# excamera/alfalfa

Hardware: AMD Instinct MI355X
Metric: 1080p macroblocks/s decode (bit-exact vs reference) (higher is better)
Workload: dtype u8

## Files before the change

__graft_entry__.py:

```python
import os
import subprocess
import sys

ROOT = os.path.dirname(os.path.abspath(__file__))
for p in (ROOT, os.path.join(ROOT, "oracle")):
    if p not in sys.path:
        sys.path.insert(0, p)


def build():
    from alfalfa_amd import build as b
    b.build(force=True, verbose=True)
    subprocess.run(["make", "-C", os.path.join(ROOT, "oracle"), "liboracle.so"], check=True)
    if os.path.isdir("/root/reference/src/decoder"):
        subprocess.run(["make", "-j8", "-C", os.path.join(ROOT, "oracle"), "ref"], check=True)
    import alfalfa_amd
    from alfalfa_amd import capi
    capi.lib()
    dont_write = sys.dont_write_bytecode
    sys.dont_write_bytecode = True
    try:
        sys.path.insert(0, os.path.join(ROOT, "tests"))
        import test_gpu_stages
        test_gpu_stages.build_stage_lib()
        if os.path.isdir("/root/reference/src/frontend"):
            import test_reference_callers as rc
            rc.build_callers(); rc.build_state_check(); rc.build_two_step()
    finally:
        sys.dont_write_bytecode = dont_write


def smoke():
    import alfalfa_amd as aa
    import vp8_oracle as vo
    path = os.path.join(ROOT, "tests", "golden", "qcif_q30_lf24.ivf")
    w, h, frames = aa.read_ivf(path)
    ctx = aa.Context(0)
    dec = aa.Decoder(ctx, w, h)
    ora = vo.OracleDecoder(w, h)
    for i, fr in enumerate(frames[:3]):
        shown, fi = dec.get_frame_output(fr)
        ora.decode(fr)
        assert dec.raster_bytes(fi) == ora.raster_bytes(), "HIP path differs from the oracle at frame %d" % i
    print("smoke ok: %d frames, %dx%d, bit-exact vs oracle" % (3, w, h))


if __name__ == "__main__":
    build()
    if "--smoke" in sys.argv:
        smoke()
```

alfalfa_amd/csrc/coeff_pack.hh:

```
#pragma once
#include "tok_fsm.hh"

namespace aa {
namespace pack {

constexpr uint64_t kInvZigzagNib = tok::nib( { 0, 1, 5, 6, 2, 4, 7, 12, 3, 8, 11, 13, 9, 10, 14, 15 } );
constexpr bool inverse_ok()
{
  for ( unsigned k = 0; k < 16; k++ )
    if ( ( ( kInvZigzagNib >> ( 4 * ( ( tok::kZigzagNib >> ( 4 * k ) ) & 15u ) ) ) & 15u ) != k ) return false;
  return true;
}
static_assert( inverse_ok(), "kInvZigzagNib is not the inverse of the zigzag scan" );

AA_HD inline uint32_t popc( uint32_t v )
{
#if defined( __HIP_DEVICE_COMPILE__ )
  return static_cast<uint32_t>( __popc( v ) );
#else
  return static_cast<uint32_t>( __builtin_popcount( v ) );
#endif
}

AA_HD inline uint32_t blocks_of( uint32_t nz_mask ) { return popc( nz_mask & 0x01FFFFFFu ); }

constexpr uint32_t kMaskSlots = 25;
AA_HD inline uint32_t zigzag_of( uint32_t j ) { return static_cast<uint32_t>( kInvZigzagNib >> ( 4 * j ) ) & 15u; }
template <class P> AA_HD inline int16_t value_at( uint32_t mask, P v, uint32_t j )
{
  const uint32_t k = zigzag_of( j );
  if ( !( ( mask >> k ) & 1u ) ) return 0;
  return static_cast<int16_t>( v[popc( mask & ( ( 1u << k ) - 1u ) )] );
}
AA_HD inline uint32_t parse_order_block( uint32_t p ) { return p == 0 ? 24u : p - 1u; }

template <class L> AA_HD inline size_t word_offset( uint32_t pos, L list )
{
  return static_cast<size_t>( list[1u + ( pos >> 15 )] ) * kChunkWords + ( pos & ( kChunkWords - 1u ) );
}

inline uint32_t expand_macroblock( const int16_t * words, uint32_t nz_mask, int16_t * dense )
{
  if ( !( nz_mask & 0x01FFFFFFu ) ) return 0;
  const int16_t * v = words + kMaskSlots;
  uint32_t n = 0;
  for ( uint32_t p = 0; p < 25; p++ ) {
    const uint32_t b = parse_order_block( p );
    if ( !( ( nz_mask >> b ) & 1u ) ) continue;
    const uint32_t mask = static_cast<uint16_t>( words[b] );
    for ( uint32_t j = 0; j < 16; j++ ) dense[16 * n + j] = value_at( mask, v, j );
    v += popc( mask );
    n++;
  }
  return static_cast<uint32_t>( v - words );
}

}
}
```

alfalfa_amd/csrc/kernels.hip:

```cpp
#include <hip/hip_runtime.h>
#include <algorithm>
#include <cstddef>

#include <cstdlib>

#include "device_types.h"
#include "vp8_math.hh"
#include "coeff_pack.hh"
#include "recon_inl.hh"

namespace aa {
namespace {
using namespace recon;

constexpr int kLanes = 64;

enum : int { DC_PRED, V_PRED, H_PRED, TM_PRED, B_PRED, NEARESTMV, NEARMV, ZEROMV, NEWMV, SPLITMV };

struct alignas( 16 ) ResidualLds {
  union {
    int16_t cf[25][16];
    int16_t res[24][16];
  };
  int16_t im[24][16];
// ... 579 lines not shown
    const int gy = cy0 - 4 + r, gx = cx0 - 4 + d * 4;
    uint32_t v = 0;
    if ( gy >= 0 && gx >= 0 ) v = *reinterpret_cast<const uint32_t *>( f.cur[1 + pl] + static_cast<size_t>( gy ) * cw + gx );
    *reinterpret_cast<uint32_t *>( &L.c[pl][r][d * 4] ) = v;
  }
  __syncthreads();

  lf_passes( L, col > 0, row > 0, !( mb.flags & AA_MB_LF_SKIP_INNER ), P, lane );

  for ( int i = lane; i < 100; i += kLanes ) {
    const int r = i / 5, d = i % 5;
    const int gy = y0 - 4 + r, gx = x0 - 4 + d * 4;
    if ( r == 0 || gy < 0 || gx < 0 ) continue;
    if ( r < 4 && d == 0 ) continue;
    *reinterpret_cast<uint32_t *>( Y + static_cast<size_t>( gy ) * pw + gx ) = *reinterpret_cast<const uint32_t *>( &L.y[r][d * 4] );
  }
  for ( int i = lane; i < 72; i += kLanes ) {
    const int pl = i / 36, e = i % 36, r = e / 3, d = e % 3;
    const int gy = cy0 - 4 + r, gx = cx0 - 4 + d * 4;
    if ( r == 0 || gy < 0 || gx < 0 ) continue;
    if ( r < 4 && d == 0 ) continue;
    *reinterpret_cast<uint32_t *>( f.cur[1 + pl] + static_cast<size_t>( gy ) * cw + gx ) = *reinterpret_cast<const uint32_t *>( &L.c[pl][r][d * 4] );
  }
}

struct alignas( 16 ) Intra4Slot {
  alignas( 16 ) int16_t res[24][16];
  alignas( 16 ) uint8_t y[17][48];
  alignas( 16 ) uint8_t c[2][9][32];
  alignas( 16 ) int16_t y2[32];
};
struct alignas( 16 ) Intra4Lds { Intra4Slot slot[4]; uint32_t tab[160]; };

template <class Slot>
__device__ __forceinline__ void residual_x4( Slot & S, const aa_dev_frame & f, const bool has_res, const bool has_y2, const uint32_t nz_mask,
                                             const uint32_t coeff_index, const uint32_t off_hi, const int segment, const int l )
{
  if ( __any( has_res ) ) {
    const bool pk = f.packed != 0;
    const int16_t * const src = pk ? f.coeffs + ( static_cast<size_t>( off_hi ) << 32 | coeff_index ) : f.coeffs + static_cast<size_t>( coeff_index ) * 16;
    const uint16_t * const q = f.quant[segment];
    const bool y2_stored = has_y2 && ( ( nz_mask >> 24 ) & 1u );
    uint32_t vbase = pack::kMaskSlots;
    if ( __any( y2_stored ) ) {
      if ( y2_stored ) {
        if ( pk ) {
          const uint32_t m24 = static_cast<uint16_t>( src[24] );
          const uint32_t zz = pack::zigzag_of( static_cast<uint32_t>( l ) );
          const int c = ( ( m24 >> zz ) & 1u ) ? src[pack::kMaskSlots + __popc( m24 & ( ( 1u << zz ) - 1u ) )] : 0;
          S.y2[l] = static_cast<int16_t>( dequant( c, q[l ? 3 : 2] ) );
          vbase += __popc( m24 );
        } else S.y2[l] = static_cast<int16_t>( dequant( src[l], q[l ? 3 : 2] ) );
      }
      __syncthreads();
      if ( y2_stored && l < 4 ) {
        const Quad v = iwht_pass1( S.y2[l], S.y2[l + 4], S.y2[l + 8], S.y2[l + 12] );
        S.y2[16 + l] = static_cast<int16_t>( v.v0 ); S.y2[16 + l + 4] = static_cast<int16_t>( v.v1 );
        S.y2[16 + l + 8] = static_cast<int16_t>( v.v2 ); S.y2[16 + l + 12] = static_cast<int16_t>( v.v3 );
      }
      __syncthreads();
      if ( y2_stored && l < 4 ) {
        const int o = l * 4;
        const Quad v = iwht_pass2( S.y2[16 + o], S.y2[16 + o + 1], S.y2[16 + o + 2], S.y2[16 + o + 3] );
        S.y2[o] = static_cast<int16_t>( v.v0 ); S.y2[o + 1] = static_cast<int16_t>( v.v1 );
        S.y2[o + 2] = static_cast<int16_t>( v.v2 ); S.y2[o + 3] = static_cast<int16_t>( v.v3 );
      }
      __syncthreads();
    }
#pragma unroll
    for ( int round = 0; round < 2; round++ ) {
      const int blk = round == 0 ? l : 16 + ( l & 7 );
      const bool mine = has_res && ( round == 0 || l < 8 );
      const bool stored = mine && ( ( nz_mask >> blk ) & 1u );
      const bool wht_dc = round == 0 && has_y2;
      const int dc = ( wht_dc && y2_stored ) ? S.y2[blk] : 0;
      if ( !__any( mine ) ) continue;
      if ( __any( stored ) ) {
        uint32_t d[8] = { 0, 0, 0, 0, 0, 0, 0, 0 };
        const uint32_t pmask = ( stored && pk ) ? static_cast<uint16_t>( src[blk] ) : 0u;
        const int pcount = __popc( pmask ), pincl = slot_scan16( pcount );
        if ( __any( stored && pk ) ) load_packed_block( pmask, src + vbase + ( pincl - pcount ), d );
        vbase += static_cast<uint32_t>( __shfl( pincl, 15, 16 ) );
        if ( stored && !pk ) {
          const uint4 * p = reinterpret_cast<const uint4 *>( src + ( __popc( nz_mask & ( ( 1u << blk ) - 1u ) ) + static_cast<int>( nz_mask >> 24 ) ) * 16 );
          const uint4 a = p[0], b = p[1];
          d[0] = a.x; d[1] = a.y; d[2] = a.z; d[3] = a.w; d[4] = b.x; d[5] = b.y; d[6] = b.z; d[7] = b.w;
        }
        const int base = round == 0 ? 0 : 4;
        int r[16];
        idct_block_regs( d, q[base], q[base + 1], wht_dc, dc, r );
        if ( mine ) {
          uint32_t o[8];
#pragma unroll
          for ( int i = 0; i < 8; i++ ) o[i] = ( static_cast<uint32_t>( r[2 * i] ) & 0xFFFFu ) | ( static_cast<uint32_t>( r[2 * i + 1] ) << 16 );
          uint4 * dst = reinterpret_cast<uint4 *>( &S.res[blk][0] );
          dst[0] = make_uint4( o[0], o[1], o[2], o[3] ); dst[1] = make_uint4( o[4], o[5], o[6], o[7] );
        }
      } else if ( mine ) {
        const pk2 v = pk_splat( ( static_cast<int16_t>( dc ) + 4 ) >> 3 );
        uint4 * dst = reinterpret_cast<uint4 *>( &S.res[blk][0] );
        dst[0] = make_uint4( v, v, v, v ); dst[1] = make_uint4( v, v, v, v );
      }
    }
  }
}

__device__ __forceinline__ uint32_t bigpred_x4( const int mode, const uint32_t above, const int left, const int corner, const int dc, const bool has_res, const int16_t * res )
{
  uint32_t out = 0;
#pragma unroll
  for ( int j = 0; j < 4; j++ ) {
    int v = bigpred_pixel( mode, ( above >> ( 8 * j ) ) & 0xFF, left, corner, dc );
    if ( has_res ) v = clamp255( v + res[j] );
    out |= static_cast<uint32_t>( v ) << ( 8 * j );
  }
  return out;
}

__device__ __forceinline__ void recon_intra4_row( const aa_frame_list & list, const int group, const int row, const int mbh_max, aa_sync_ws * ws, Intra4Lds & L,
                                                  const int home_xcc )
{
  const int lane = threadIdx.x, slot = lane >> 4, l = lane & 15;
  Intra4Slot & S = L.slot[slot];
  const aa_dev_frame * const fp = list.f[group * 4 + slot];
  const aa_dev_frame & f = fp ? *fp : *list.f[group * 4];
  const bool frame_on = fp != nullptr && row < fp->mbh;
  const int mbw = f.mbw, pw = mbw * 16, cw = pw >> 1;
  const int y0 = row * 16, cy0 = row * 8;
  int * const progress = ws->progress + ( group * 4 + slot ) * mbh_max;
  uint8_t * const Y = f.cur[0];
  uint8_t * const Cl = f.cur[1 + ( l >> 3 )];
  const int words = ( frame_on && f.has_intra ) ? ( mbw + 63 ) >> 6 : 0;
  const unsigned long long * const mask = f.intra_rows + static_cast<size_t>( row ) * ( ( mbw + 63 ) >> 6 );
  int w = 0;
  unsigned long long m = words ? mask[0] : 0ull;
  bool row_done = false;
  int seen = row > 0 ? 0 : 0x7FFFFFFF;

  for ( ;; ) {
    while ( m == 0 && w + 1 < words ) { ++w; m = mask[w]; }
    const bool on = m != 0;
    if ( !__any( on ) ) break;
    const int col = on ? w * 64 + __ffsll( static_cast<long long>( m ) ) - 1 : 0;
    m &= m - 1;
    publish_progress( frame_on && l == 0 && ( on || !row_done ), &progress[row], on ? col : mbw );
    row_done = row_done || !on;

    const aa_mb_info * const mb = f.mbs + static_cast<size_t>( row ) * mbw + col;
    uint4 hd = make_uint4( 0, 0, 0, 0 ), bm = make_uint4( 0, 0, 0, 0 );
    if ( on ) { hd = *reinterpret_cast<const uint4 *>( mb ); bm = *reinterpret_cast<const uint4 *>( mb->u.b_mode ); }
    const int y_mode = hd.x & 0xFF, uv_mode = ( hd.x >> 8 ) & 0xFF, segment = ( hd.x >> 24 ) & 3, flags = hd.y & 0xFF;
    const uint32_t nz_mask = hd.z, coeff_index = hd.w;
    const bool has_res = on && ( flags & AA_MB_HAS_NONZERO );
    const bool has_y2 = has_res && ( flags & AA_MB_HAS_Y2 );
    const int need = min( col + 2, mbw );
    if ( on && row > 0 && seen < need ) seen = poll_progress( &progress[row - 1] );

    residual_x4( S, f, has_res, has_y2, nz_mask, coeff_index, hd.y >> 24, segment, l );

    if ( row > 0 ) wait_for_row_above( on, need, seen, 1, ws, progress, group, row, mbh_max, home_xcc, kMinPolls, kMaxWaitTicks );
    const int x0 = col * 16, cx0 = col * 8;
    if ( on ) {
      if ( l < 6 ) {
        uint32_t v;
        const uint8_t * a = Y + static_cast<size_t>( y0 - 1 ) * pw;
        if ( y0 == 0 ) v = 0x7F7F7F7Fu;
        else if ( l == 0 ) v = x0 > 0 ? load_u32<true>( a + x0 - 4 ) : 0x81818181u;
        else if ( l <= 4 ) v = load_u32<true>( a + x0 + ( l - 1 ) * 4 );
        else if ( x0 + 16 >= pw ) v = 0x01010101u * ( load_u32<true>( a + pw - 4 ) >> 24 );
        else v = load_u32<true>( a + x0 + 16 );
        *reinterpret_cast<uint32_t *>( &S.y[0][12 + l * 4] ) = v;
      } else if ( l < 12 ) {
        const int pl = ( l - 6 ) / 3, i = ( l - 6 ) % 3;
        const uint8_t * a = f.cur[1 + pl] + static_cast<size_t>( cy0 - 1 ) * cw;
        uint32_t v;
        if ( cy0 == 0 ) v = 0x7F7F7F7Fu;
        else if ( i == 0 ) v = cx0 > 0 ? load_u32<true>( a + cx0 - 4 ) : 0x81818181u;
        else v = load_u32<true>( a + cx0 + ( i - 1 ) * 4 );
        *reinterpret_cast<uint32_t *>( &S.c[pl][0][12 + i * 4] ) = v;
      }
      S.y[l + 1][15] = x0 > 0 ? static_cast<uint8_t>( load_u32<true>( Y + static_cast<size_t>( y0 + l ) * pw + x0 - 4 ) >> 24 ) : 129;
      S.c[l >> 3][( l & 7 ) + 1][15] = cx0 > 0 ? static_cast<uint8_t>( load_u32<true>( Cl + static_cast<size_t>( cy0 + ( l & 7 ) ) * cw + cx0 - 4 ) >> 24 ) : 129;
    }
    __syncthreads();

    if ( on ) {
      const int pl = l >> 3, r = l & 7;
      const uint32_t a0 = *reinterpret_cast<const uint32_t *>( &S.c[pl][0][16] ), a1 = *reinterpret_cast<const uint32_t *>( &S.c[pl][0][20] );
      const int sa = absdiff_sum4( a0 ) + absdiff_sum4( a1 );
      int sl = 0;
#pragma unroll
// ... 64 lines not shown
      packed |= ( idx < 4 ? ( 4 - idx ) * 48 : idx - 4 ) << ( 8 * k );
      packed |= ( idx >= 9 ? 1u : 0u ) << ( 24 + k );
    }
    L.tab[i] = packed;
  }
  const int xcc = xcc_id();
  if ( xcc >= n_xcd ) { if ( threadIdx.x == 0 ) atomicExch( &ws->error, 3 ); return; }
  for ( ;; ) {
    const int t = take_ticket( ws, xcc, &s_ticket, threadIdx.x );
    const int mine = xcc < n_groups ? ( n_groups - xcc + n_xcd - 1 ) / n_xcd : 0;
    if ( t >= mine * mbh_max ) return;
    recon_intra4_row( list, ( t % mine ) * n_xcd + xcc, t / mine, mbh_max, ws, L, xcc );
  }
}

struct alignas( 16 ) Inter4Slot {
  alignas( 16 ) int16_t res[24][16];
  union {
    struct {
      alignas( 16 ) uint8_t wy[21][24];
      uint8_t wc[2][13][16];
    };
    alignas( 16 ) uint8_t pred[384];
  };
  union {
    alignas( 16 ) uint8_t ty[16][24];
    alignas( 16 ) int16_t y2[32];
  };
  alignas( 16 ) uint8_t tc[2][8][16];
};
struct alignas( 16 ) Inter4Lds { Inter4Slot slot[4]; uint32_t taps[16]; };
static_assert( offsetof( Inter4Slot, wc ) == offsetof( Inter4Slot, wy ) + 21 * 24, "wy and wc must be contiguous" );

__device__ __forceinline__ void recon_inter4_body( const aa_dev_frame & f, const unsigned bq, const unsigned max_quads, Inter4Lds & L )
{
  const int lane = threadIdx.x, slot = lane >> 4, l = lane & 15;
  Inter4Slot & S = L.slot[slot];
  if ( lane < 16 ) {
    uint32_t a, b; pack_taps( lane >> 1, a, b ); L.taps[lane] = ( lane & 1 ) ? b : a;
  }
  const unsigned total = static_cast<unsigned>( f.mbw ) * f.mbh;
  const unsigned chunk = ( max_quads + 7u ) >> 3;
  const unsigned qi = ( bq & 7u ) * chunk + ( bq >> 3 );
  const unsigned mi = qi * 4u + slot;
  const int mbw = f.mbw, pw = mbw * 16, ph = f.mbh * 16, cw = pw >> 1, ch = ph >> 1;
  bool on = qi < max_quads && mi < total;
  const aa_mb_info * const mb = f.mbs + ( on ? mi : 0u );
  uint4 hd = make_uint4( 0, 0, 0, 0 ); uint32_t mvw = 0;
  if ( on ) { hd = *reinterpret_cast<const uint4 *>( mb ); mvw = *reinterpret_cast<const uint32_t *>( &mb->u.mv[0][0] ); }
  const int y_mode = hd.x & 0xFF, ref_frame = ( hd.x >> 16 ) & 3, segment = ( hd.x >> 24 ) & 3, flags = hd.y & 0xFF;
  const uint32_t nz_mask = hd.z, coeff_index = hd.w;
  on = on && ( flags & AA_MB_INTER ) && y_mode != SPLITMV;
  if ( !__any( on ) ) return;
  const int col = on ? static_cast<int>( mi % static_cast<unsigned>( mbw ) ) : 0, row = on ? static_cast<int>( mi / static_cast<unsigned>( mbw ) ) : 0;
  const bool has_res = on && ( flags & AA_MB_HAS_NONZERO );
  const bool has_y2 = has_res && ( flags & AA_MB_HAS_Y2 );
  const uint8_t * const * ref = f.ref[on ? ref_frame : 1];
  const uint8_t * const ref_y = ref[0], * const ref_u = ref[1], * const ref_v = ref[2];
  const int mvx = static_cast<int16_t>( mvw & 0xFFFFu ), mvy = static_cast<int>( mvw ) >> 16;
  const int cmx = chroma_mv( 4 * mvx ), cmy = chroma_mv( 4 * mvy );
  const int sxy = col * 16 + ( mvx >> 3 ) - 2, syy = row * 16 + ( mvy >> 3 ) - 2;
  const int sxc = col * 8 + ( cmx >> 3 ) - 2, syc = row * 8 + ( cmy >> 3 ) - 2;
  const int axy = sxy & ~3, axc = sxc & ~3;
  const bool inside = sxy >= 0 && syy >= 0 && axy + 24 <= pw && syy + 21 <= ph && sxc >= 0 && syc >= 0 && axc + 16 <= cw && syc + 13 <= ch;
  const bool fast = on && inside;
  uint32_t wreg[15];
  const int l6 = l / 6, lm = l - 6 * l6;
  const uint8_t * const wy0 = ref_y + static_cast<ptrdiff_t>( syy ) * pw + axy;
  const uint8_t * const wu0 = ref_u + static_cast<ptrdiff_t>( syc ) * cw + axc;
  const uint8_t * const wv0 = ref_v + static_cast<ptrdiff_t>( syc ) * cw + axc;
#pragma unroll
  for ( int k = 0; k < 15; k++ ) {
    const int i = l + 16 * k;
    wreg[k] = 0;
    if ( fast ) {
      if ( k < 7 || ( k == 7 && i < 126 ) ) {
        const int carry = lm + ( 4 * k ) % 6 >= 6 ? 1 : 0;
        const int r = l6 + 2 * k + ( 4 * k ) / 6 + carry, d = lm + ( 4 * k ) % 6 - 6 * carry;
        wreg[k] = *reinterpret_cast<const uint32_t *>( wy0 + static_cast<ptrdiff_t>( r ) * pw + d * 4 );
      } else if ( i < 230 ) {
        const int j = i - 126, pl = j >= 52 ? 1 : 0, e = j - 52 * pl;
        wreg[k] = *reinterpret_cast<const uint32_t *>( ( pl ? wv0 : wu0 ) + static_cast<ptrdiff_t>( e >> 2 ) * cw + ( e & 3 ) * 4 );
      }
    }
  }

  residual_x4( S, f, has_res, has_y2, nz_mask, coeff_index, hd.y >> 24, segment, l );

  {
    uint32_t * flat = reinterpret_cast<uint32_t *>( &S.wy[0][0] );
    if ( fast ) {
#pragma unroll
      for ( int k = 0; k < 15; k++ ) { const int i = l + 16 * k; if ( i < 230 ) flat[i] = wreg[k]; }
    }
    if ( __any( on && !inside ) ) {
      if ( on && !inside ) {
        uint8_t * by = &S.wy[0][0];
        for ( int i = l; i < 21 * 24; i += 16 ) {
          const int r = i / 24, c = i % 24;
          by[i] = ref_y[static_cast<size_t>( clampi( syy + r, 0, ph - 1 ) ) * pw + clampi( sxy + c, 0, pw - 1 )];
        }
        uint8_t * bc = &S.wc[0][0][0];
        for ( int i = l; i < 2 * 13 * 16; i += 16 ) {
          const int pl = i / 208, e = i % 208, r = e >> 4, c = e & 15;
          bc[i] = ( pl ? ref_v : ref_u )[static_cast<size_t>( clampi( syc + r, 0, ch - 1 ) ) * cw + clampi( sxc + c, 0, cw - 1 )];
        }
      }
    }
  }
  const int oy = inside ? ( sxy & 3 ) : 0, oc = inside ? ( sxc & 3 ) : 0;
  __syncthreads();

  const bool luma_general = __any( on && ( ( mvx | mvy ) & 7 ) != 0 ), chroma_general = __any( on && ( ( cmx | cmy ) & 7 ) != 0 );
  const uint8_t * const wyb = &S.wy[0][0]; const uint8_t * const wcb = &S.wc[0][0][0];
  uint8_t * const tyb = &S.ty[0][0]; uint8_t * const tcb = &S.tc[0][0][0];
  if ( on && luma_general ) {
    const int frac = mvx & 7;
    const uint32_t t0 = L.taps[2 * frac], t1 = L.taps[2 * frac + 1];
#pragma unroll
    for ( int k = 0; k < 6; k++ ) {
// ... 44 lines not shown
    const int frac = mvy & 7;
    const uint32_t t0 = L.taps[2 * frac], t1 = L.taps[2 * frac + 1];
#pragma unroll
    for ( int k = 0; k < 4; k++ ) {
      const int t = l + 16 * k, c = t >> 2, i = t & 3;
      const uint8_t * sp = tyb + c * 24 + i * 4;
      const uint32_t o4 = sixtap_x4_lane( *reinterpret_cast<const uint32_t *>( sp ), *reinterpret_cast<const uint32_t *>( sp + 4 ), *reinterpret_cast<const uint32_t *>( sp + 8 ), 0, frac, t0, t1 );
      uint8_t * pb = S.pred + ( i * 4 ) * 16 + c;
      pb[0] = static_cast<uint8_t>( o4 ); pb[16] = static_cast<uint8_t>( o4 >> 8 ); pb[32] = static_cast<uint8_t>( o4 >> 16 ); pb[48] = static_cast<uint8_t>( o4 >> 24 );
    }
  }
  if ( on && chroma_general ) {
    const int frac = cmy & 7;
    const uint32_t t0 = L.taps[2 * frac], t1 = L.taps[2 * frac + 1];
#pragma unroll
    for ( int k = 0; k < 2; k++ ) {
      const int j = l + 16 * k, pl = j >> 4, c = ( j >> 1 ) & 7, i = j & 1;
      const uint8_t * sp = tcb + pl * 128 + c * 16 + i * 4;
      const uint32_t o4 = sixtap_x4_lane( *reinterpret_cast<const uint32_t *>( sp ), *reinterpret_cast<const uint32_t *>( sp + 4 ), *reinterpret_cast<const uint32_t *>( sp + 8 ), 0, frac, t0, t1 );
      uint8_t * pb = S.pred + 256 + pl * 64 + ( i * 4 ) * 8 + c;
      pb[0] = static_cast<uint8_t>( o4 ); pb[8] = static_cast<uint8_t>( o4 >> 8 ); pb[16] = static_cast<uint8_t>( o4 >> 16 ); pb[24] = static_cast<uint8_t>( o4 >> 24 );
    }
  }
  __syncthreads();

  if ( on ) {
    uint32_t o[4];
#pragma unroll
    for ( int k = 0; k < 4; k++ ) {
      const uint32_t p4 = *reinterpret_cast<const uint32_t *>( S.pred + l * 16 + 4 * k );
      const uint32_t out = has_res ? add_residual_x4( p4, &S.res[( l >> 2 ) * 4 + k][( l & 3 ) * 4] ) : p4;
      o[k] = out;
    }
    *reinterpret_cast<uint4 *>( f.cur[0] + static_cast<size_t>( row * 16 + l ) * pw + col * 16 ) = make_uint4( o[0], o[1], o[2], o[3] );
    const int pl = l >> 3, r = l & 7;
    uint32_t oc2[2];
#pragma unroll
    for ( int k = 0; k < 2; k++ ) {
      const uint32_t p4 = *reinterpret_cast<const uint32_t *>( S.pred + 256 + pl * 64 + r * 8 + 4 * k );
      const uint32_t out = has_res ? add_residual_x4( p4, &S.res[16 + pl * 4 + ( r >> 2 ) * 2 + k][( r & 3 ) * 4] ) : p4;
      oc2[k] = out;
    }
    *reinterpret_cast<uint2 *>( f.cur[1 + pl] + static_cast<size_t>( row * 8 + r ) * cw + col * 8 ) = make_uint2( oc2[0], oc2[1] );
  }
}

__global__ __launch_bounds__( kLanes ) void k_recon_inter4( const aa_frame_list list, const unsigned max_quads )
{
  __builtin_amdgcn_s_setprio( 3 );

  __shared__ Inter4Lds L;
  recon_inter4_body( *list.f[blockIdx.y], blockIdx.x, max_quads, L );
}

constexpr int kStripMbs = 8;
constexpr int kStripRow = 16 + 16 * kStripMbs;
constexpr int kStripRpi = 16 / kStripMbs;
static_assert( ( kStripRow / 16 ) % 2 == 1, "odd multiple of 16: consecutive rows start on different banks" );
struct alignas( 16 ) LfStrip {
  uint8_t c[12][kStripRow];
  uint8_t y[20][kStripRow];
  uint8_t halo_y[16][4];
  uint8_t halo_c[2][8][4];
  uint8_t pad[32];
};
struct alignas( 16 ) LfStripLds { LfStrip slot[4]; };

__device__ __forceinline__ uint64_t load_u64_shared( const uint8_t * p )
{
  return __hip_atomic_load( reinterpret_cast<const uint64_t *>( p ), __ATOMIC_RELAXED, __HIP_MEMORY_SCOPE_AGENT );
}

__device__ __forceinline__ void lf_edges_pk( pk2 ( &v )[20], const LfParamsPk & P, const pk2 g0, const pk2 g1, const pk2 g23 )
{
  if ( __any( g0 != 0u ) ) lf_edge_pk( P, true, g0, v[0], v[1], v[2], v[3], v[4], v[5], v[6], v[7] );
  if ( __any( g1 != 0u ) ) {
    lf_edge_pk( P, false, g1, v[4], v[5], v[6], v[7], v[8], v[9], v[10], v[11] );
    if ( __any( g23 != 0u ) ) {
      lf_edge_pk( P, false, g23, v[8], v[9], v[10], v[11], v[12], v[13], v[14], v[15] );
      lf_edge_pk( P, false, g23, v[12], v[13], v[14], v[15], v[16], v[17], v[18], v[19] );
    }
  }
}

__device__ __forceinline__ void loopfilter_strip_row( const aa_frame_list & list, const int group, const int row, const int mbh_max, const int mbw_max,
// ... 479 lines not shown
```

alfalfa_amd/csrc/recon_inl.hh:

```
#pragma once
#include <hip/hip_runtime.h>

#include "vp8_math.hh"
#include "coeff_pack.hh"

namespace aa {
namespace recon {

__device__ __forceinline__ void pack_taps( const int frac, uint32_t & t0123, uint32_t & t45 )
{
  t0123 = ( sixtap_coeff( frac, 0 ) & 0xFF ) | ( ( sixtap_coeff( frac, 1 ) & 0xFF ) << 8 ) | ( ( sixtap_coeff( frac, 2 ) & 0xFF ) << 16 )
          | ( static_cast<uint32_t>( sixtap_coeff( frac, 3 ) & 0xFF ) << 24 );
  t45 = ( sixtap_coeff( frac, 4 ) & 0xFF ) | ( ( sixtap_coeff( frac, 5 ) & 0xFF ) << 8 );
}

__device__ __forceinline__ void idct_block_regs( const uint32_t ( &d )[8], const int fdc, const int fac, const bool replace_dc, const int dc, int ( &r )[16] )
{
  const pk2 fpair = pk_splat( fac ), f0 = ( static_cast<uint32_t>( fdc ) & 0xFFFFu ) | ( static_cast<uint32_t>( fac ) << 16 );
  int c[16];
#pragma unroll
  for ( int i = 0; i < 8; i++ ) {
    const pk2 m = pk_mul( d[i], i == 0 ? f0 : fpair );
    c[2 * i] = static_cast<int16_t>( m & 0xFFFFu ); c[2 * i + 1] = static_cast<int>( m ) >> 16;
  }
  if ( replace_dc ) c[0] = dc;
  int im[16];
#pragma unroll
  for ( int i = 0; i < 4; i++ ) { const Quad v = idct_pass1( c[i], c[i + 4], c[i + 8], c[i + 12] ); im[i * 4] = v.v0; im[i * 4 + 1] = v.v1; im[i * 4 + 2] = v.v2; im[i * 4 + 3] = v.v3; }
#pragma unroll
  for ( int i = 0; i < 4; i++ ) { const Quad v = idct_pass2( im[i], im[i + 4], im[i + 8], im[i + 12] ); r[i * 4] = v.v0; r[i * 4 + 1] = v.v1; r[i * 4 + 2] = v.v2; r[i * 4 + 3] = v.v3; }
}


__device__ __forceinline__ int slot_scan16( int v )
{
  v += __builtin_amdgcn_update_dpp( 0, v, 0x111, 0xF, 0xF, true );
  v += __builtin_amdgcn_update_dpp( 0, v, 0x112, 0xF, 0xF, true );
  v += __builtin_amdgcn_update_dpp( 0, v, 0x114, 0xF, 0xF, true );
  v += __builtin_amdgcn_update_dpp( 0, v, 0x118, 0xF, 0xF, true );
  return v;
}
__device__ __forceinline__ void load_packed_block( const uint32_t mask, const int16_t * const v, uint32_t ( &d )[8] )
{
#pragma unroll
  for ( int j = 0; j < 16; j++ ) {
    const uint32_t zz = static_cast<uint32_t>( pack::kInvZigzagNib >> ( 4 * j ) ) & 15u;
    const bool there = ( mask >> zz ) & 1u;
    if ( !__any( there ) ) continue;
    uint32_t c = 0;
    if ( there ) c = static_cast<uint16_t>( v[__popc( mask & ( ( 1u << zz ) - 1u ) )] );
    d[j >> 1] |= c << ( 16 * ( j & 1 ) );
  }
}


__device__ __forceinline__ uint32_t sixtap_x4_lane( const uint32_t d0, const uint32_t d1, const uint32_t d2, const int o, const int frac, const uint32_t t0123, const uint32_t t45 )
{
  const uint32_t w0 = __builtin_amdgcn_alignbyte( d1, d0, o ), w1 = __builtin_amdgcn_alignbyte( d2, d1, o ), w2 = __builtin_amdgcn_alignbyte( 0u, d2, o );
  const uint32_t ident = __builtin_amdgcn_alignbyte( w1, w0, 2 );
  const uint32_t b0 = w0 ^ 0x80808080u, b1 = w1 ^ 0x80808080u, b2 = w2 ^ 0x80808080u;
  int v[4];
#pragma unroll
  for ( int k = 0; k < 4; k++ ) {
    const int a = static_cast<int>( __builtin_amdgcn_alignbyte( b1, b0, k ) ), b = static_cast<int>( __builtin_amdgcn_alignbyte( b2, b1, k ) );
    v[k] = __builtin_amdgcn_sdot4( a, static_cast<int>( t0123 ), __builtin_amdgcn_sdot4( b, static_cast<int>( t45 ), 16384 + 64, false ), false );
  }
  const uint32_t lo = __builtin_amdgcn_ashr_pk_u8_i32( v[0], v[1], 7 ), hi = __builtin_amdgcn_ashr_pk_u8_i32( v[2], v[3], 7 );
  const uint32_t out = __builtin_amdgcn_perm( hi, lo, 0x05040100u );
  return frac == 0 ? ident : out;
}

__device__ __forceinline__ uint32_t add_residual_x4( const uint32_t p4, const int16_t * res )
{
  const uint2 r = *reinterpret_cast<const uint2 *>( res );
  const pk2 s0 = pk_add( __builtin_amdgcn_perm( 0u, p4, 0x0c010c00u ), r.x ), s1 = pk_add( __builtin_amdgcn_perm( 0u, p4, 0x0c030c02u ), r.y );
  uint32_t b0, b1;
  asm( "v_sat_pk_u8_i16 %0, %1" : "=v"( b0 ) : "v"( s0 ) );
  asm( "v_sat_pk_u8_i16 %0, %1" : "=v"( b1 ) : "v"( s1 ) );
  return b0 | ( b1 << 16 );
}


}
}
// ... 1 lines not shown
```

Measured before the change: 124.9 million.

## Batch residual coefficient loads ahead of Y2 WHT and use wave-held frame descriptor

Restructures residual_x4 so that the luma, chroma and Y2 coefficient masks are fetched early and all coefficient loads for both rounds are issued together before the WHT barriers. This lets global-load latency overlap instead of serialising per round. The inter kernel now loads the frame descriptor with one dword per lane and extracts fields with readlane, and accesses use explicit global address-space pointers. This raises register pressure (two 16-entry coefficient arrays held live) and adds a new test build step.

```diff
diff --git a/__graft_entry__.py b/__graft_entry__.py
--- a/__graft_entry__.py
+++ b/__graft_entry__.py
@@ -23,6 +23,8 @@
         sys.path.insert(0, os.path.join(ROOT, "tests"))
         import test_gpu_stages
         test_gpu_stages.build_stage_lib()
+        import test_gpu_residual_loads
+        test_gpu_residual_loads.build_residual_stage_lib()
         if os.path.isdir("/root/reference/src/frontend"):
             import test_reference_callers as rc
             rc.build_callers(); rc.build_state_check(); rc.build_two_step()
diff --git a/alfalfa_amd/csrc/coeff_pack.hh b/alfalfa_amd/csrc/coeff_pack.hh
--- a/alfalfa_amd/csrc/coeff_pack.hh
+++ b/alfalfa_amd/csrc/coeff_pack.hh
@@ -32,6 +32,12 @@
   if ( !( ( mask >> k ) & 1u ) ) return 0;
   return static_cast<int16_t>( v[popc( mask & ( ( 1u << k ) - 1u ) )] );
 }
+constexpr uint32_t kNoValue = 0xFFFFFFFFu;
+AA_HD inline uint32_t value_index( uint32_t mask, uint32_t j )
+{
+  const uint32_t k = zigzag_of( j );
+  return ( ( mask >> k ) & 1u ) ? popc( mask & ( ( 1u << k ) - 1u ) ) : kNoValue;
+}
 AA_HD inline uint32_t parse_order_block( uint32_t p ) { return p == 0 ? 24u : p - 1u; }
 
 template <class L> AA_HD inline size_t word_offset( uint32_t pos, L list )
diff --git a/alfalfa_amd/csrc/kernels.hip b/alfalfa_amd/csrc/kernels.hip
--- a/alfalfa_amd/csrc/kernels.hip
+++ b/alfalfa_amd/csrc/kernels.hip
@@ -635,79 +635,6 @@
 };
 struct alignas( 16 ) Intra4Lds { Intra4Slot slot[4]; uint32_t tab[160]; };
 
-template <class Slot>
-__device__ __forceinline__ void residual_x4( Slot & S, const aa_dev_frame & f, const bool has_res, const bool has_y2, const uint32_t nz_mask,
-                                             const uint32_t coeff_index, const uint32_t off_hi, const int segment, const int l )
-{
-  if ( __any( has_res ) ) {
-    const bool pk = f.packed != 0;
-    const int16_t * const src = pk ? f.coeffs + ( static_cast<size_t>( off_hi ) << 32 | coeff_index ) : f.coeffs + static_cast<size_t>( coeff_index ) * 16;
-    const uint16_t * const q = f.quant[segment];
-    const bool y2_stored = has_y2 && ( ( nz_mask >> 24 ) & 1u );
-    uint32_t vbase = pack::kMaskSlots;
-    if ( __any( y2_stored ) ) {
-      if ( y2_stored ) {
-        if ( pk ) {
-          const uint32_t m24 = static_cast<uint16_t>( src[24] );
-          const uint32_t zz = pack::zigzag_of( static_cast<uint32_t>( l ) );
-          const int c = ( ( m24 >> zz ) & 1u ) ? src[pack::kMaskSlots + __popc( m24 & ( ( 1u << zz ) - 1u ) )] : 0;
-          S.y2[l] = static_cast<int16_t>( dequant( c, q[l ? 3 : 2] ) );
-          vbase += __popc( m24 );
-        } else S.y2[l] = static_cast<int16_t>( dequant( src[l], q[l ? 3 : 2] ) );
-      }
-      __syncthreads();
-      if ( y2_stored && l < 4 ) {
-        const Quad v = iwht_pass1( S.y2[l], S.y2[l + 4], S.y2[l + 8], S.y2[l + 12] );
-        S.y2[16 + l] = static_cast<int16_t>( v.v0 ); S.y2[16 + l + 4] = static_cast<int16_t>( v.v1 );
-        S.y2[16 + l + 8] = static_cast<int16_t>( v.v2 ); S.y2[16 + l + 12] = static_cast<int16_t>( v.v3 );
-      }
-      __syncthreads();
-      if ( y2_stored && l < 4 ) {
-        const int o = l * 4;
-        const Quad v = iwht_pass2( S.y2[16 + o], S.y2[16 + o + 1], S.y2[16 + o + 2], S.y2[16 + o + 3] );
-        S.y2[o] = static_cast<int16_t>( v.v0 ); S.y2[o + 1] = static_cast<int16_t>( v.v1 );
-        S.y2[o + 2] = static_cast<int16_t>( v.v2 ); S.y2[o + 3] = static_cast<int16_t>( v.v3 );
-      }
-      __syncthreads();
-    }
-#pragma unroll
-    for ( int round = 0; round < 2; round++ ) {
-      const int blk = round == 0 ? l : 16 + ( l & 7 );
-      const bool mine = has_res && ( round == 0 || l < 8 );
-      const bool stored = mine && ( ( nz_mask >> blk ) & 1u );
-      const bool wht_dc = round == 0 && has_y2;
-      const int dc = ( wht_dc && y2_stored ) ? S.y2[blk] : 0;
-      if ( !__any( mine ) ) continue;
-      if ( __any( stored ) ) {
-        uint32_t d[8] = { 0, 0, 0, 0, 0, 0, 0, 0 };
-        const uint32_t pmask = ( stored && pk ) ? static_cast<uint16_t>( src[blk] ) : 0u;
-        const int pcount = __popc( pmask ), pincl = slot_scan16( pcount );
-        if ( __any( stored && pk ) ) load_packed_block( pmask, src + vbase + ( pincl - pcount ), d );
-        vbase += static_cast<uint32_t>( __shfl( pincl, 15, 16 ) );
-        if ( stored && !pk ) {
-          const uint4 * p = reinterpret_cast<const uint4 *>( src + ( __popc( nz_mask & ( ( 1u << blk ) - 1u ) ) + static_cast<int>( nz_mask >> 24 ) ) * 16 );
-          const uint4 a = p[0], b = p[1];
-          d[0] = a.x; d[1] = a.y; d[2] = a.z; d[3] = a.w; d[4] = b.x; d[5] = b.y; d[6] = b.z; d[7] = b.w;
-        }
-        const int base = round == 0 ? 0 : 4;
-        int r[16];
-        idct_block_regs( d, q[base], q[base + 1], wht_dc, dc, r );
-        if ( mine ) {
-          uint32_t o[8];
-#pragma unroll
-          for ( int i = 0; i < 8; i++ ) o[i] = ( static_cast<uint32_t>( r[2 * i] ) & 0xFFFFu ) | ( static_cast<uint32_t>( r[2 * i + 1] ) << 16 );
-          uint4 * dst = reinterpret_cast<uint4 *>( &S.res[blk][0] );
-          dst[0] = make_uint4( o[0], o[1], o[2], o[3] ); dst[1] = make_uint4( o[4], o[5], o[6], o[7] );
-        }
-      } else if ( mine ) {
-        const pk2 v = pk_splat( ( static_cast<int16_t>( dc ) + 4 ) >> 3 );
-        uint4 * dst = reinterpret_cast<uint4 *>( &S.res[blk][0] );
-        dst[0] = make_uint4( v, v, v, v ); dst[1] = make_uint4( v, v, v, v );
-      }
-    }
-  }
-}
-
 __device__ __forceinline__ uint32_t bigpred_x4( const int mode, const uint32_t above, const int left, const int corner, const int dc, const bool has_res, const int16_t * res )
 {
   uint32_t out = 0;
@@ -726,22 +653,24 @@
   const int lane = threadIdx.x, slot = lane >> 4, l = lane & 15;
   Intra4Slot & S = L.slot[slot];
   const aa_dev_frame * const fp = list.f[group * 4 + slot];
-  const aa_dev_frame & f = fp ? *fp : *list.f[group * 4];
-  const bool frame_on = fp != nullptr && row < fp->mbh;
+  const AA_GLOBAL aa_dev_frame & f = *as_global( fp ? fp : list.f[group * 4] );
+  const bool frame_on = fp != nullptr && row < f.mbh;
   const int mbw = f.mbw, pw = mbw * 16, cw = pw >> 1;
+  const aa_mb_info * const mbs = f.mbs;
+  const AA_GLOBAL uint32_t * const quant = reinterpret_cast<const AA_GLOBAL uint32_t *>( &f.quant[0][0] );
   const int y0 = row * 16, cy0 = row * 8;
   int * const progress = ws->progress + ( group * 4 + slot ) * mbh_max;
   uint8_t * const Y = f.cur[0];
   uint8_t * const Cl = f.cur[1 + ( l >> 3 )];
   const int words = ( frame_on && f.has_intra ) ? ( mbw + 63 ) >> 6 : 0;
-  const unsigned long long * const mask = f.intra_rows + static_cast<size_t>( row ) * ( ( mbw + 63 ) >> 6 );
+  const auto mask_word = [&]( const int i ) { return as_global( f.intra_rows )[static_cast<size_t>( row ) * ( ( mbw + 63 ) >> 6 ) + i]; };
   int w = 0;
-  unsigned long long m = words ? mask[0] : 0ull;
+  unsigned long long m = words ? mask_word( 0 ) : 0ull;
   bool row_done = false;
   int seen = row > 0 ? 0 : 0x7FFFFFFF;
 
   for ( ;; ) {
-    while ( m == 0 && w + 1 < words ) { ++w; m = mask[w]; }
+    while ( m == 0 && w + 1 < words ) { ++w; m = mask_word( w ); }
     const bool on = m != 0;
     if ( !__any( on ) ) break;
     const int col = on ? w * 64 + __ffsll( static_cast<long long>( m ) ) - 1 : 0;
@@ -749,9 +678,10 @@
     publish_progress( frame_on && l == 0 && ( on || !row_done ), &progress[row], on ? col : mbw );
     row_done = row_done || !on;
 
-    const aa_mb_info * const mb = f.mbs + static_cast<size_t>( row ) * mbw + col;
+    const AA_GLOBAL aa_mb_info * const mb = as_global( mbs + static_cast<size_t>( row ) * mbw + col );
     uint4 hd = make_uint4( 0, 0, 0, 0 ), bm = make_uint4( 0, 0, 0, 0 );
-    if ( on ) { hd = *reinterpret_cast<const uint4 *>( mb ); bm = *reinterpret_cast<const uint4 *>( mb->u.b_mode ); }
+    const int16_t * const coeffs = f.coeffs; const bool pk = f.packed != 0;
+    if ( on ) hd = *reinterpret_cast<const AA_GLOBAL uint4 *>( mb );
     const int y_mode = hd.x & 0xFF, uv_mode = ( hd.x >> 8 ) & 0xFF, segment = ( hd.x >> 24 ) & 3, flags = hd.y & 0xFF;
     const uint32_t nz_mask = hd.z, coeff_index = hd.w;
     const bool has_res = on && ( flags & AA_MB_HAS_NONZERO );
@@ -759,7 +689,12 @@
     const int need = min( col + 2, mbw );
     if ( on && row > 0 && seen < need ) seen = poll_progress( &progress[row - 1] );
 
-    residual_x4( S, f, has_res, has_y2, nz_mask, coeff_index, hd.y >> 24, segment, l );
+    {
+      const ResidualRequest rq = residual_request( coeffs, pk, has_res, has_y2, nz_mask, coeff_index, hd.y >> 24, l );
+      const Quant3 q = { quant[3 * segment], quant[3 * segment + 1], quant[3 * segment + 2] };
+      residual_x4( S, rq, pk, q, has_res, has_y2, nz_mask, l );
+    }
+    if ( on ) bm = *reinterpret_cast<const AA_GLOBAL uint4 *>( mb->u.b_mode );
 
     if ( row > 0 ) wait_for_row_above( on, need, seen, 1, ws, progress, group, row, mbh_max, home_xcc, kMinPolls, kMaxWaitTicks );
     const int x0 = col * 16, cx0 = col * 8;
@@ -890,22 +825,29 @@
 struct alignas( 16 ) Inter4Lds { Inter4Slot slot[4]; uint32_t taps[16]; };
 static_assert( offsetof( Inter4Slot, wc ) == offsetof( Inter4Slot, wy ) + 21 * 24, "wy and wc must be contiguous" );
 
-__device__ __forceinline__ void recon_inter4_body( const aa_dev_frame & f, const unsigned bq, const unsigned max_quads, Inter4Lds & L )
+__device__ __forceinline__ void recon_inter4_body( const aa_dev_frame * const fp, const unsigned bq, const unsigned max_quads, Inter4Lds & L )
 {
   const int lane = threadIdx.x, slot = lane >> 4, l = lane & 15;
   Inter4Slot & S = L.slot[slot];
-  if ( lane < 16 ) {
-    uint32_t a, b; pack_taps( lane >> 1, a, b ); L.taps[lane] = ( lane & 1 ) ? b : a;
-  }
-  const unsigned total = static_cast<unsigned>( f.mbw ) * f.mbh;
+  const WaveHeld<aa_dev_frame> F( fp, lane );
+  const uint32_t geometry = F.u32( offsetof( aa_dev_frame, mbw ) );
+  static_assert( offsetof( aa_dev_frame, mbh ) == offsetof( aa_dev_frame, mbw ) + 2 && offsetof( aa_dev_frame, mbw ) % 4 == 0, "mbw | mbh << 16 is one dword" );
+  const int mbw = geometry & 0xFFFFu, mbh = geometry >> 16;
+  {
+    uint32_t w = 0;
+#pragma unroll
+    for ( int k = 0; k < 16; k++ ) { uint32_t a, b; pack_taps( k >> 1, a, b ); w = lane == k ? ( ( k & 1 ) ? b : a ) : w; }
+    if ( lane < 16 ) L.taps[lane] = w;
+  }
+  const unsigned total = static_cast<unsigned>( mbw ) * mbh;
   const unsigned chunk = ( max_quads + 7u ) >> 3;
   const unsigned qi = ( bq & 7u ) * chunk + ( bq >> 3 );
   const unsigned mi = qi * 4u + slot;
-  const int mbw = f.mbw, pw = mbw * 16, ph = f.mbh * 16, cw = pw >> 1, ch = ph >> 1;
+  const int pw = mbw * 16, ph = mbh * 16, cw = pw >> 1, ch = ph >> 1;
   bool on = qi < max_quads && mi < total;
-  const aa_mb_info * const mb = f.mbs + ( on ? mi : 0u );
+  const AA_GLOBAL aa_mb_info * const mb = as_global( F.ptr<const aa_mb_info>( offsetof( aa_dev_frame, mbs ) ) + ( on ? mi : 0u ) );
   uint4 hd = make_uint4( 0, 0, 0, 0 ); uint32_t mvw = 0;
-  if ( on ) { hd = *reinterpret_cast<const uint4 *>( mb ); mvw = *reinterpret_cast<const uint32_t *>( &mb->u.mv[0][0] ); }
+  if ( on ) { mvw = *reinterpret_cast<const AA_GLOBAL uint32_t *>( &mb->u.mv[0][0] ); hd = *reinterpret_cast<const AA_GLOBAL uint4 *>( mb ); }
   const int y_mode = hd.x & 0xFF, ref_frame = ( hd.x >> 16 ) & 3, segment = ( hd.x >> 24 ) & 3, flags = hd.y & 0xFF;
   const uint32_t nz_mask = hd.z, coeff_index = hd.w;
   on = on && ( flags & AA_MB_INTER ) && y_mode != SPLITMV;
@@ -913,8 +855,19 @@
   const int col = on ? static_cast<int>( mi % static_cast<unsigned>( mbw ) ) : 0, row = on ? static_cast<int>( mi / static_cast<unsigned>( mbw ) ) : 0;
   const bool has_res = on && ( flags & AA_MB_HAS_NONZERO );
   const bool has_y2 = has_res && ( flags & AA_MB_HAS_Y2 );
-  const uint8_t * const * ref = f.ref[on ? ref_frame : 1];
-  const uint8_t * const ref_y = ref[0], * const ref_u = ref[1], * const ref_v = ref[2];
+  const int rf = on ? ref_frame : 1;
+  const auto plane = [&]( const int p ) {
+    const auto r = [&]( const int k ) { return F.ptr<const uint8_t>( offsetof( aa_dev_frame, ref ) + ( 3 * k + p ) * sizeof( uint8_t * ) ); };
+    return as_global( rf < 2 ? ( rf == 0 ? r( 0 ) : r( 1 ) ) : ( rf == 2 ? r( 2 ) : r( 3 ) ) );
+  };
+  const AA_GLOBAL uint8_t * const ref_y = plane( 0 ), * const ref_u = plane( 1 ), * const ref_v = plane( 2 );
+  const auto quant = [&]( const int k ) {
+    const auto w = [&]( const int i ) { return F.u32( offsetof( aa_dev_frame, quant ) + 4 * i ); };
+    const uint32_t q0 = w( k ), q1 = w( 3 + k ), q2 = w( 6 + k ), q3 = w( 9 + k );
+    return segment < 2 ? ( segment == 0 ? q0 : q1 ) : ( segment == 2 ? q2 : q3 );
+  };
+  const bool pk = F.u32( offsetof( aa_dev_frame, packed ) ) != 0;
+  const ResidualRequest rq = residual_request( F.ptr<const int16_t>( offsetof( aa_dev_frame, coeffs ) ), pk, has_res, has_y2, nz_mask, coeff_index, hd.y >> 24, l );
   const int mvx = static_cast<int16_t>( mvw & 0xFFFFu ), mvy = static_cast<int>( mvw ) >> 16;
   const int cmx = chroma_mv( 4 * mvx ), cmy = chroma_mv( 4 * mvy );
   const int sxy = col * 16 + ( mvx >> 3 ) - 2, syy = row * 16 + ( mvy >> 3 ) - 2;
@@ -924,9 +877,9 @@
   const bool fast = on && inside;
   uint32_t wreg[15];
   const int l6 = l / 6, lm = l - 6 * l6;
-  const uint8_t * const wy0 = ref_y + static_cast<ptrdiff_t>( syy ) * pw + axy;
-  const uint8_t * const wu0 = ref_u + static_cast<ptrdiff_t>( syc ) * cw + axc;
-  const uint8_t * const wv0 = ref_v + static_cast<ptrdiff_t>( syc ) * cw + axc;
+  const AA_GLOBAL uint8_t * const wy0 = ref_y + static_cast<ptrdiff_t>( syy ) * pw + axy;
+  const AA_GLOBAL uint8_t * const wu0 = ref_u + static_cast<ptrdiff_t>( syc ) * cw + axc;
+  const AA_GLOBAL uint8_t * const wv0 = ref_v + static_cast<ptrdiff_t>( syc ) * cw + axc;
 #pragma unroll
   for ( int k = 0; k < 15; k++ ) {
     const int i = l + 16 * k;
@@ -935,15 +888,15 @@
       if ( k < 7 || ( k == 7 && i < 126 ) ) {
         const int carry = lm + ( 4 * k ) % 6 >= 6 ? 1 : 0;
         const int r = l6 + 2 * k + ( 4 * k ) / 6 + carry, d = lm + ( 4 * k ) % 6 - 6 * carry;
-        wreg[k] = *reinterpret_cast<const uint32_t *>( wy0 + static_cast<ptrdiff_t>( r ) * pw + d * 4 );
+        wreg[k] = *reinterpret_cast<const AA_GLOBAL uint32_t *>( wy0 + static_cast<ptrdiff_t>( r ) * pw + d * 4 );
       } else if ( i < 230 ) {
         const int j = i - 126, pl = j >= 52 ? 1 : 0, e = j - 52 * pl;
-        wreg[k] = *reinterpret_cast<const uint32_t *>( ( pl ? wv0 : wu0 ) + static_cast<ptrdiff_t>( e >> 2 ) * cw + ( e & 3 ) * 4 );
-      }
-    }
-  }
-
-  residual_x4( S, f, has_res, has_y2, nz_mask, coeff_index, hd.y >> 24, segment, l );
+        wreg[k] = *reinterpret_cast<const AA_GLOBAL uint32_t *>( ( pl ? wv0 : wu0 ) + static_cast<ptrdiff_t>( e >> 2 ) * cw + ( e & 3 ) * 4 );
+      }
+    }
+  }
+
+  residual_x4( S, rq, pk, Quant3 { quant( 0 ), quant( 1 ), quant( 2 ) }, has_res, has_y2, nz_mask, l );
 
   {
     uint32_t * flat = reinterpret_cast<uint32_t *>( &S.wy[0][0] );
@@ -1054,7 +1007,7 @@
       const uint32_t out = has_res ? add_residual_x4( p4, &S.res[( l >> 2 ) * 4 + k][( l & 3 ) * 4] ) : p4;
       o[k] = out;
     }
-    *reinterpret_cast<uint4 *>( f.cur[0] + static_cast<size_t>( row * 16 + l ) * pw + col * 16 ) = make_uint4( o[0], o[1], o[2], o[3] );
+    *reinterpret_cast<uint4 *>( F.ptr<uint8_t>( offsetof( aa_dev_frame, cur ) ) + static_cast<size_t>( row * 16 + l ) * pw + col * 16 ) = make_uint4( o[0], o[1], o[2], o[3] );
     const int pl = l >> 3, r = l & 7;
     uint32_t oc2[2];
 #pragma unroll
@@ -1063,7 +1016,8 @@
       const uint32_t out = has_res ? add_residual_x4( p4, &S.res[16 + pl * 4 + ( r >> 2 ) * 2 + k][( r & 3 ) * 4] ) : p4;
       oc2[k] = out;
     }
-    *reinterpret_cast<uint2 *>( f.cur[1 + pl] + static_cast<size_t>( row * 8 + r ) * cw + col * 8 ) = make_uint2( oc2[0], oc2[1] );
+    uint8_t * const cu = F.ptr<uint8_t>( offsetof( aa_dev_frame, cur ) + sizeof( uint8_t * ) ), * const cv = F.ptr<uint8_t>( offsetof( aa_dev_frame, cur ) + 2 * sizeof( uint8_t * ) );
+    *reinterpret_cast<uint2 *>( ( pl ? cv : cu ) + static_cast<size_t>( row * 8 + r ) * cw + col * 8 ) = make_uint2( oc2[0], oc2[1] );
   }
 }
 
@@ -1072,7 +1026,7 @@
   __builtin_amdgcn_s_setprio( 3 );
 
   __shared__ Inter4Lds L;
-  recon_inter4_body( *list.f[blockIdx.y], blockIdx.x, max_quads, L );
+  recon_inter4_body( list.f[blockIdx.y], blockIdx.x, max_quads, L );
 }
 
 constexpr int kStripMbs = 8;
diff --git a/alfalfa_amd/csrc/recon_inl.hh b/alfalfa_amd/csrc/recon_inl.hh
--- a/alfalfa_amd/csrc/recon_inl.hh
+++ b/alfalfa_amd/csrc/recon_inl.hh
@@ -40,16 +40,154 @@
   v += __builtin_amdgcn_update_dpp( 0, v, 0x118, 0xF, 0xF, true );
   return v;
 }
+template <class T> __device__ __forceinline__ const AA_GLOBAL T * as_global( const T * p ) { return (const AA_GLOBAL T *) p; }
+
+template <class T> struct WaveHeld {
+  static_assert( sizeof( T ) <= 64 * 4 && sizeof( T ) % 4 == 0, "one dword per lane" );
+  uint32_t dw;
+  __device__ __forceinline__ WaveHeld( const T * p, const int lane ) : dw( as_global( reinterpret_cast<const uint32_t *>( p ) )[static_cast<unsigned>( lane ) < sizeof( T ) / 4 ? lane : 0] ) {}
+  __device__ __forceinline__ uint32_t u32( const size_t byte_offset ) const { return static_cast<uint32_t>( __builtin_amdgcn_readlane( static_cast<int>( dw ), static_cast<int>( byte_offset / 4 ) ) ); }
+  template <class P> __device__ __forceinline__ P * ptr( const size_t byte_offset ) const
+  {
+    return reinterpret_cast<P *>( static_cast<uintptr_t>( u32( byte_offset ) ) | static_cast<uintptr_t>( u32( byte_offset + 4 ) ) << 32 );
+  }
+};
+
+__device__ __forceinline__ void request_packed_block( const uint32_t mask, const int16_t * const v, uint32_t ( &c )[16] )
+{
+  const AA_GLOBAL int16_t * const g = as_global( v );
+#pragma unroll
+  for ( int j = 0; j < 16; j++ ) {
+    const uint32_t i = pack::value_index( mask, static_cast<uint32_t>( j ) );
+    const bool there = i != pack::kNoValue;
+    c[j] = 0;
+    if ( !__any( there ) ) continue;
+    if ( there ) c[j] = static_cast<uint16_t>( g[i] );
+  }
+}
+__device__ __forceinline__ void requests_end_here( uint32_t ( &c )[16] )
+{
+  asm volatile( "" : "+v"( c[0] ), "+v"( c[1] ), "+v"( c[2] ), "+v"( c[3] ), "+v"( c[4] ), "+v"( c[5] ), "+v"( c[6] ), "+v"( c[7] ),
+                     "+v"( c[8] ), "+v"( c[9] ), "+v"( c[10] ), "+v"( c[11] ), "+v"( c[12] ), "+v"( c[13] ), "+v"( c[14] ), "+v"( c[15] ) );
+}
+__device__ __forceinline__ void place_packed_block( const uint32_t ( &c )[16], uint32_t ( &d )[8] )
+{
+#pragma unroll
+  for ( int j = 0; j < 16; j++ ) d[j >> 1] |= c[j] << ( 16 * ( j & 1 ) );
+}
 __device__ __forceinline__ void load_packed_block( const uint32_t mask, const int16_t * const v, uint32_t ( &d )[8] )
 {
-#pragma unroll
-  for ( int j = 0; j < 16; j++ ) {
-    const uint32_t zz = static_cast<uint32_t>( pack::kInvZigzagNib >> ( 4 * j ) ) & 15u;
-    const bool there = ( mask >> zz ) & 1u;
-    if ( !__any( there ) ) continue;
-    uint32_t c = 0;
-    if ( there ) c = static_cast<uint16_t>( v[__popc( mask & ( ( 1u << zz ) - 1u ) )] );
-    d[j >> 1] |= c << ( 16 * ( j & 1 ) );
+  uint32_t c[16];
+  request_packed_block( mask, v, c );
+  place_packed_block( c, d );
+}
+
+struct Quant3 { uint32_t y, y2, uv; };
+
+struct ResidualRequest {
+  const AA_GLOBAL int16_t * src;
+  uint32_t m_luma, m_chroma, m_y2;
+};
+__device__ __forceinline__ ResidualRequest residual_request( const int16_t * const coeffs, const bool pk, const bool has_res, const bool has_y2, const uint32_t nz_mask,
+                                                             const uint32_t coeff_index, const uint32_t off_hi, const int l )
+{
+  ResidualRequest R;
+  R.src = as_global( pk ? coeffs + ( static_cast<size_t>( off_hi ) << 32 | coeff_index ) : coeffs + static_cast<size_t>( coeff_index ) * 16 );
+  R.m_luma = R.m_chroma = R.m_y2 = 0;
+  if ( has_res && pk ) {
+    if ( ( nz_mask >> l ) & 1u ) R.m_luma = static_cast<uint16_t>( R.src[l] );
+    if ( l < 8 && ( ( nz_mask >> ( 16 + l ) ) & 1u ) ) R.m_chroma = static_cast<uint16_t>( R.src[16 + l] );
+    if ( has_y2 && ( ( nz_mask >> 24 ) & 1u ) ) R.m_y2 = static_cast<uint16_t>( R.src[24] );
+  }
+  return R;
+}
+
+template <class Slot>
+__device__ __forceinline__ void residual_x4( Slot & S, const ResidualRequest & R, const bool pk, const Quant3 q, const bool has_res, const bool has_y2,
+                                             const uint32_t nz_mask, const int l )
+{
+  if ( !__any( has_res ) ) return;
+  const AA_GLOBAL int16_t * const src = R.src;
+  const int16_t * const words = (const int16_t *) src;
+  const bool y2_stored = has_y2 && ( ( nz_mask >> 24 ) & 1u );
+  const bool stored0 = has_res && ( ( nz_mask >> l ) & 1u ), stored1 = has_res && l < 8 && ( ( nz_mask >> ( 16 + l ) ) & 1u );
+  const uint32_t pm2 = ( y2_stored && pk ) ? R.m_y2 : 0u, pm0 = ( stored0 && pk ) ? R.m_luma : 0u, pm1 = ( stored1 && pk ) ? R.m_chroma : 0u;
+  const int n0 = __popc( pm0 ), n1 = __popc( pm1 );
+  const int incl0 = slot_scan16( n0 ), incl1 = slot_scan16( n1 );
+  const uint32_t vbase = pack::kMaskSlots + static_cast<uint32_t>( __popc( pm2 ) );
+  const uint32_t first0 = vbase + static_cast<uint32_t>( incl0 - n0 ), first1 = vbase + static_cast<uint32_t>( __shfl( incl0, 15, 16 ) + incl1 - n1 );
+  uint32_t c0[16], c1[16];
+  const bool any0 = __any( stored0 ), any1 = __any( stored1 );
+  if ( any0 ) request_packed_block( pm0, words + first0, c0 );
+  if ( any1 ) request_packed_block( pm1, words + first1, c1 );
+  const bool dense0 = stored0 && !pk, dense1 = stored1 && !pk;
+  if ( __any( has_res && !pk ) ) {
+    const int before = static_cast<int>( nz_mask >> 24 );
+    if ( dense0 ) {
+      const AA_GLOBAL uint4 * p = reinterpret_cast<const AA_GLOBAL uint4 *>( src + ( __popc( nz_mask & ( ( 1u << l ) - 1u ) ) + before ) * 16 );
+      const uint4 a = p[0], b = p[1];
+      c0[0] = a.x; c0[1] = a.y; c0[2] = a.z; c0[3] = a.w; c0[4] = b.x; c0[5] = b.y; c0[6] = b.z; c0[7] = b.w;
+    }
+    if ( dense1 ) {
+      const AA_GLOBAL uint4 * p = reinterpret_cast<const AA_GLOBAL uint4 *>( src + ( __popc( nz_mask & ( ( 1u << ( 16 + l ) ) - 1u ) ) + before ) * 16 );
+      const uint4 a = p[0], b = p[1];
+      c1[0] = a.x; c1[1] = a.y; c1[2] = a.z; c1[3] = a.w; c1[4] = b.x; c1[5] = b.y; c1[6] = b.z; c1[7] = b.w;
+    }
+  }
+  int y2c = 0;
+  {
+    const uint32_t i = pack::value_index( pm2, static_cast<uint32_t>( l ) );
+    if ( y2_stored && ( !pk || i != pack::kNoValue ) ) y2c = src[pk ? pack::kMaskSlots + i : static_cast<uint32_t>( l )];
+  }
+  if ( any0 ) requests_end_here( c0 );
+  if ( any1 ) requests_end_here( c1 );
+  asm volatile( "" : "+v"( y2c ) );
+  if ( __any( y2_stored ) ) {
+    if ( y2_stored ) S.y2[l] = static_cast<int16_t>( dequant( y2c, static_cast<int>( l ? q.y2 >> 16 : q.y2 & 0xFFFFu ) ) );
+    __syncthreads();
+    if ( y2_stored && l < 4 ) {
+      const Quad v = iwht_pass1( S.y2[l], S.y2[l + 4], S.y2[l + 8], S.y2[l + 12] );
+      S.y2[16 + l] = static_cast<int16_t>( v.v0 ); S.y2[16 + l + 4] = static_cast<int16_t>( v.v1 );
+      S.y2[16 + l + 8] = static_cast<int16_t>( v.v2 ); S.y2[16 + l + 12] = static_cast<int16_t>( v.v3 );
+    }
+    __syncthreads();
+    if ( y2_stored && l < 4 ) {
+      const int o = l * 4;
+      const Quad v = iwht_pass2( S.y2[16 + o], S.y2[16 + o + 1], S.y2[16 + o + 2], S.y2[16 + o + 3] );
+      S.y2[o] = static_cast<int16_t>( v.v0 ); S.y2[o + 1] = static_cast<int16_t>( v.v1 );
+      S.y2[o + 2] = static_cast<int16_t>( v.v2 ); S.y2[o + 3] = static_cast<int16_t>( v.v3 );
+    }
+    __syncthreads();
+  }
+#pragma unroll
+  for ( int round = 0; round < 2; round++ ) {
+    const int blk = round == 0 ? l : 16 + ( l & 7 );
+    const bool mine = has_res && ( round == 0 || l < 8 );
+    const bool dense = round == 0 ? dense0 : dense1;
+    const bool wht_dc = round == 0 && has_y2;
+    const int dc = ( wht_dc && y2_stored ) ? S.y2[blk] : 0;
+    if ( !__any( mine ) ) continue;
+    if ( round == 0 ? any0 : any1 ) {
+      uint32_t d[8] = { 0, 0, 0, 0, 0, 0, 0, 0 };
+      const uint32_t ( &c )[16] = round == 0 ? c0 : c1;
+      place_packed_block( c, d );
+#pragma unroll
+      for ( int i = 0; i < 8; i++ ) d[i] = dense ? c[i] : d[i];
+      const uint32_t qq = round == 0 ? q.y : q.uv;
+      int r[16];
+      idct_block_regs( d, static_cast<int>( qq & 0xFFFFu ), static_cast<int>( qq >> 16 ), wht_dc, dc, r );
+      if ( mine ) {
+        uint32_t o[8];
+#pragma unroll
+        for ( int i = 0; i < 8; i++ ) o[i] = ( static_cast<uint32_t>( r[2 * i] ) & 0xFFFFu ) | ( static_cast<uint32_t>( r[2 * i + 1] ) << 16 );
+        uint4 * dst = reinterpret_cast<uint4 *>( &S.res[blk][0] );
+        dst[0] = make_uint4( o[0], o[1], o[2], o[3] ); dst[1] = make_uint4( o[4], o[5], o[6], o[7] );
+      }
+    } else if ( mine ) {
+      const pk2 v = pk_splat( ( static_cast<int16_t>( dc ) + 4 ) >> 3 );
+      uint4 * dst = reinterpret_cast<uint4 *>( &S.res[blk][0] );
+      dst[0] = make_uint4( v, v, v, v ); dst[1] = make_uint4( v, v, v, v );
+    }
   }
 }
 
```

Result: no change. 128.2 million (median of 6 runs) (+2.6%).
